# POSTECH-CVLab/InstaOrder

Measured on AMD Instinct MI355X. Metric: instance-pairs/sec (fwd+bwd), higher is better.
Workload: dtype f32; 1 GPU; InstaOrderNet_o, pair-batch 256 per GPU at 256x256x5, fp32, fwd+bwd+SGD (BASELINE.json configs[1]); inputs=resident in HBM, pairs_per_gpu=256, input_size=256, parallelism=dp1, hip_graph=True, setup_steps=0, inputs_distinct=True

## Files before the change

include/instaorder_hip.h:

```cpp
#ifndef INSTAORDER_HIP_H
#define INSTAORDER_HIP_H

#include <stddef.h>
#include <stdint.h>

#ifdef __cplusplus
extern "C" {
#endif

#define IO_OK 0
#define IO_ERR_SHAPE (-1)
#define IO_ERR_WORKSPACE (-2)
#define IO_ERR_LAUNCH (-3)
#define IO_ERR_STATE (-4)
#define IO_ERR_NODEVICE (-5)

#if !defined(__HIP__) && !defined(HIP_INCLUDE_HIP_HIP_RUNTIME_API_H)
typedef void* hipStream_t;
#endif

int io_abi_version(void);
const char* io_last_error_string(void);
int io_device_count(void);
int io_set_winograd(int on);
// ... 227 lines not shown

size_t io_bn_tile_partial_floats(int M, int C, int G);
int io_bn_bwd_coefs_dt(const void* dz, const void* y, int M, int C, int G, const float* gamma, const float* mean,
                       const float* rstd, float* dgamma, float* dbeta, float* coef, float* partial,
                       size_t partial_floats, int dtype, hipStream_t stream);
int io_bn_bwd_coefs_from_tile_partials(float* p1, float* p2, int M, int C, int G, const float* gamma, const float* mean,
                                       const float* rstd, float* dgamma, float* dbeta, float* coef, hipStream_t stream);
typedef struct io_dgrad_fused {
    const void* xb_y;
    const float* xb_coef;
    void* xb_dy_out;
    const void* add;
    const void* relu_mask;
    const void* ep_y;
    const float *ep_mean, *ep_rstd, *ep_scale, *ep_shift;
    void* ep_act_out;
    float *ep_p1, *ep_p2;
    float* wino_scratch;
    size_t wino_scratch_floats;
    const uint32_t* relu_maskbits;
} io_dgrad_fused;
int io_conv2d_dgrad_fused_dt(const void* dy, const void* wt, void* dx, int N, int H, int W, int Cin, int Cout, int R,
                             int S, int pad, int G, const io_dgrad_fused* f, int dtype, hipStream_t stream);
size_t io_conv2d_wino_scratch_floats(int Cin, int Cout);
int io_conv2d_fwd_wino(const float* x, const float* w, float* y, int N, int H, int W, int Cin, int Cout, int G,
                       const float* in_mean, const float* in_scale, const float* in_shift, const float* gamma,
                       const float* beta, float* running_mean, float* running_var, float momentum, float eps, float* mean,
                       float* rstd, float* scale, float* shift, float* workspace, size_t workspace_floats,
                       float* wino_scratch, size_t wino_floats, hipStream_t stream);
int io_conv2d_fwd_xf_dt(const void* x, const void* w, void* y, int N, int H, int W, int Cin, int Cout, int R, int S,
                        int stride, int pad, int G, const float* in_mean, const float* in_scale, const float* in_shift,
                        const float* gamma, const float* beta, float* running_mean, float* running_var, float momentum, float eps,
                        float* mean, float* rstd, float* scale, float* shift, float* workspace, size_t workspace_floats,
                        int dtype, hipStream_t stream);
int io_conv2d_fwd_resid(const float* y3, const float* identity, const float* w, float* y, float* out, int N, int H, int W,
                        int Cin, int Cout, int G, const float* in_mean, const float* in_scale, const float* in_shift,
                        const float* gamma, const float* beta, float* running_mean, float* running_var, float momentum,
                        float eps, float* mean, float* rstd, float* scale, float* shift, float* workspace,
                        size_t workspace_floats, hipStream_t stream);
int io_conv2d_fwd_resid_dt(const void* y3, const void* second, const void* w, void* y, void* out, uint32_t* out_bits, int N,
                           int H, int W, int Cin, int Cout, int G, int two, const float* ta, const float* tb, const float* tc,
                           float* tile_mean, float* tile_m2, int dtype, hipStream_t stream);
int io_set_bf16_p256_xop(int on);
int io_get_bf16_p256_xop(void);
typedef struct io_weight_desc {
    long src, dst_op, dst_t, dst_g;
// ... 176 lines not shown
```

instaorder_amd/_lib.py:

```python
import ctypes as C
import os

_HERE = os.path.dirname(os.path.abspath(__file__))
LIB_PATH = os.environ.get("IO_LIB_PATH") or os.path.join(_HERE, "libinstaorder_hip.so")
_lib = None

c_float_p = C.c_void_p


def csrc_digest():
    import glob
    import hashlib
    h = hashlib.sha256()
    files = sorted(glob.glob(os.path.join(_HERE, "csrc", "*.hip")) + glob.glob(os.path.join(_HERE, "csrc", "*.h")))
    files.append(os.path.join(os.path.dirname(_HERE), "include", "instaorder_hip.h"))
    for f in files:
        h.update(os.path.basename(f).encode())
        h.update(open(f, "rb").read())
    return h.hexdigest()[:16]


class TensorInfo(C.Structure):
    _fields_ = [("name", C.c_char * 64), ("kind", C.c_int), ("ndim", C.c_int), ("shape", C.c_long * 4),
                ("offset", C.c_long), ("numel_storage", C.c_long), ("cin_storage", C.c_int),
# ... 176 lines not shown
                                      _P, _P, _P, _P, _Z, _I, _I, _P]),
    "io_conv2d_fwd_bias_dt": (_I, [_P, _P, _P, _I, _I, _I, _I, _I, _I, _I, _I, _I, _P, _P, _I, _I, _I, _P]),
    "io_stem_packed_floats": (_Z, [_I]),
    "io_stem_wgrad_exact_workspace_bytes": (_Z, [_I, _I, _I, _I]),
    "io_stem_fwd_bnstats_exact": (_I, [_P, _P, _P, _I, _I, _I, _I, _I, _P, _P, _P, _P, _F, _F, _P, _P, _P, _P, _P, _Z, _P,
                                       _P]),
    "io_stem_wgrad_exact": (_I, [_P, _P, _P, _I, _I, _I, _I, _P, _Z, _P, _P]),
    "io_stem_wgrad_exact_bn": (_I, [_P, _P, _P, _P, _I, _I, _I, _I, _I, _P, _P, _P, _P, _P, _P, _P, _P, _P, _Z, _P, _Z, _P,
                                    _P]),
    "io_stem_wgrad_bn_bf16": (_I, [_P, _P, _P, _P, _I, _I, _I, _I, _P, _P, _P, _P, _P, _P, _P, _P, _P, _Z, _P, _Z, _P]),
    "io_stem_wgrad_bf16_workspace_bytes": (_Z, []),
    "io_debug_last_wgrad_route": (_I, []),
    "io_conv2d_fwd_resid": (_I, [_P, _P, _P, _P, _P, _I, _I, _I, _I, _I, _I, _P, _P, _P, _P, _P, _P, _P, _F, _F, _P, _P, _P,
                                 _P, _P, _Z, _P]),
    "io_smooth_loss_workspace_floats": (_Z, [_I, _I, _I]),
    "io_smooth_loss_fwd": (_I, [_P, _P, _I, _I, _I, _F, _P, _P, _P, _Z, _P]),
    "io_smooth_loss_bwd": (_I, [_P, _P, _P, _F, _I, _I, _I, _I, _P, _P]),
    "io_disp_order_workspace_floats": (_Z, [_I, _I, _I]),
    "io_disp_order_count": (_I, [_P, _P, _P, _P, _P, _P, _I, _I, _I, _I, _F, _P, _P, _Z, _P]),
    "io_bn_tile_partial_floats": (_Z, [_I, _I, _I]),
    "io_bn_bwd_coefs_dt": (_I, [_P, _P, _I, _I, _I, _P, _P, _P, _P, _P, _P, _P, _Z, _I, _P]),
    "io_bn_bwd_coefs_from_tile_partials": (_I, [_P, _P, _I, _I, _I, _P, _P, _P, _P, _P, _P, _P]),
    "io_conv2d_dgrad_fused_dt": (_I, [_P, _P, _P, _I, _I, _I, _I, _I, _I, _I, _I, _I, C.POINTER(DgradFused), _I, _P]),
    "io_conv2d_dgrad_bnbwd_dt": (_I, [_P, _P, _P, _I, _I, _I, _I, _I, _I, _I, _I, _P, _I, _P, _P, _P, _P, _P, _P, _P, _P, _P,
                                      _Z, _I, _I, _P]),
    "io_prof_launches": (_I, [_P, _I]),
    "io_weights_prepare": (_I, [_P, _I, _P, _P, _I, _P]),
    "io_weights_unpack_grads": (_I, [_P, _I, _P, _P, _P]),
    "io_maxpool_fwd_xf_dt": (_I, [_P, _I, _I, _I, _I, _P, _P, _I, _P, _P, _P, _I, _P]),
    "io_conv2d_fwd_xf_dt": (_I, [_P, _P, _P, _I, _I, _I, _I, _I, _I, _I, _I, _I, _I, _P, _P, _P, _P, _P, _P, _P, _F, _F, _P,
                                 _P, _P, _P, _P, _Z, _I, _P]),
    "io_conv2d_wino_scratch_floats": (_Z, [_I, _I]),
    "io_conv2d_fwd_wino": (_I, [_P, _P, _P, _I, _I, _I, _I, _I, _I, _P, _P, _P, _P, _P, _P, _P, _F, _F, _P, _P, _P, _P, _P, _Z,
                                _P, _Z, _P]),
    "io_maxpool_fwd_dt": (_I, [_P, _I, _I, _I, _I, _P, _P, _I, _P]),
    "io_maxpool_bwd_dt": (_I, [_P, _P, _I, _I, _I, _I, _P, _I, _P]),
    "io_avgpool_fc_fwd_dt": (_I, [_P, _I, _I, _I, _P, _P, _I, _P, _P, _I, _P, _P, _I, _P]),
    "io_avgpool_fc_bwd_dt": (_I, [_P, _P, _I, _I, _I, _P, _I, _P, _I, _P, _P, _P, _P, _P, _P, _I, _P]),
    "io_depth_errors_median_workspace_bytes": (_Z, [_I, _I, _I]),
    "io_depth_errors_median": (_I, [_P, _P, _I, _I, _I, _F, _F, _F, _P, _P, _P, _Z, _P]),
    "io_disp_sample_points": (_I, [_P, _I, _I, _I, _P, _P, _P, _P]),
    "io_mask_pack": (_I, [_P, _I, _I, _I, _I, _I, _P, _P, _P]),
    "io_mask_pair_counts": (_I, [_P, _I, _P, _I, _I, _I, _P, _P]),
    "io_instance_depth_select_workspace_bytes": (_Z, [_I, _I, _I]),
    "io_instance_depth_select": (_I, [_P, _I, _I, _P, _I, _I, _P, _P, _P, _P, _P, _Z, _P]),
    "io_prof_begin": (_I, []),
# ... 40 lines not shown
```

instaorder_amd/csrc/capi.hip:

```cpp
#include <stdarg.h>
#include <stdio.h>
#include <stdlib.h>
#include <string.h>

#include "io_common.h"

static thread_local char g_err[512] = "";

void io_set_error(const char* fmt, ...) {
    va_list ap;
    va_start(ap, fmt);
    vsnprintf(g_err, sizeof(g_err), fmt, ap);
    va_end(ap);
}

int io_check_launch(const char* what) {
    hipError_t e = hipGetLastError();
    if (e != hipSuccess) {
        io_set_error("%s: %s", what, hipGetErrorString(e));
        return IO_ERR_LAUNCH;
    }
    return IO_OK;
}

// ... 158 lines not shown
    return io_conv_wgrad_partial_bytes(g, Cin == 8);
}

extern "C" int io_conv2d_wgrad(const float* x, const float* dy, float* dw, int N, int H, int W, int Cin, int Cout,
                               int R, int S, int stride, int pad, void* ws, size_t ws_bytes, hipStream_t st) {
    IoConvGeom g = io_geom_fwd(N, H, W, Cin, Cout, R, S, stride, pad);
    return io_launch_conv_wgrad(g, x, dy, dw, (float*)ws, ws_bytes, Cin == 8, st);
}

#include <mutex>
#include <vector>
namespace {
struct ProfRec { int cls; double flops, bytes, fexec; hipEvent_t e0, e1; bool own0, closed; hipStream_t st; };
std::mutex g_prof_mu;
bool g_prof_on = false;
bool g_prof_share = true;
std::vector<ProfRec> g_prof_recs;
std::vector<hipEvent_t> g_prof_pool;
const char* kProfNames[IO_PROF_NCLASS] = {"conv_nt_kernel<128,false>", "conv_nt_kernel<64,false>",
    "conv_nt_kernel<64,true>", "conv_wgrad_kernel", "conv_wgrad_kernel<64,64,true>", "bn_stats_finalize",
    "bn_apply", "bn_bwd", "pool_head", "filter_transpose", "pack_planes", "order_loss", "sgd_momentum",
    "conv_nt_kernel<wino>", "conv_wgrad_kernel<wino>", "adam", "grad_norm", "rle_decode", "poly_fill",
    "jpeg_entropy", "jpeg_idct", "jpeg_colour", "jpeg_prog_entropy", "png_inflate", "png_unfilter", "png_pack",
    "png_par_search", "png_par_count", "png_par_store", "png_par_resolve"};
hipEvent_t prof_event() {
    if (!g_prof_pool.empty()) { hipEvent_t e = g_prof_pool.back(); g_prof_pool.pop_back(); return e; }
    hipEvent_t e;
    (void)hipEventCreate(&e);
    return e;
}
}

IoProfScope::IoProfScope(int cls, double flops, double bytes, hipStream_t stream, double flops_exec) : idx(-1), st(stream) {
    if (!g_prof_on) return;
    std::lock_guard<std::mutex> lk(g_prof_mu);
    if (!g_prof_on) return;
    ProfRec r;
    r.cls = cls; r.flops = flops; r.bytes = bytes; r.fexec = flops_exec < 0.0 ? flops : flops_exec;
    r.st = st; r.closed = false;
    if (g_prof_share && !g_prof_recs.empty() && g_prof_recs.back().closed && g_prof_recs.back().st == st) {
        r.e0 = g_prof_recs.back().e1;
        r.own0 = false;
    } else {
        r.e0 = prof_event();
        r.own0 = true;
        (void)hipEventRecord(r.e0, st);
    }
// ... 483 lines not shown
```

instaorder_amd/csrc/conv_igemm.hip:

```cpp
#include <string.h>
#include <stdlib.h>

#include "io_common.h"

namespace {

constexpr int kThreads = 256;

__device__ __forceinline__ f32x4 ld4(const float* p) { return *reinterpret_cast<const f32x4*>(p); }
template <typename T> __device__ __forceinline__ void pin(T& v) { asm volatile("" : "+v"(v)); }
__device__ __forceinline__ void st4(float* p, f32x4 v) { *reinterpret_cast<f32x4*>(p) = v; }

__device__ __forceinline__ int xcd_remap(int b, int nwg) {
    const int q = nwg >> 3, r = nwg & 7, x = b & 7, i = b >> 3;
    return (x < r ? x * (q + 1) : r * (q + 1) + (x - r) * q) + i;
}

__device__ __forceinline__ int sdiv(int n, float rd) { return (int)(((float)n + 0.5f) * rd); }
__device__ __forceinline__ int stem_kp(int wT, int cr) { return (wT * cr + 31) / 32 * 32; }
__device__ __forceinline__ int fdiv(int n, IoFastDiv f) {
    return f.shift < 0 ? n : (int)(__umulhi((unsigned)n, f.magic) >> f.shift);
}

typedef unsigned u32x4 __attribute__((ext_vector_type(4)));
// ... 2497 lines not shown

size_t io_conv_wgrad_partial_bytes(const IoConvGeom& g, int stem) {
    const int s0 = plan_wgrad(g, stem, true).splits, s1 = plan_wgrad(g, stem, false).splits;
    int splits = s0 > s1 ? s0 : s1;
    if (wgrad_wino_shape_ok(g, stem)) {
        const int sw = plan_wgrad_wino(g).splits;
        if (sw > splits) splits = sw;
    }
    size_t need = splits == 1 ? 0 : (size_t)splits * g.Co * io_filter_row(g) * sizeof(float);
    if (stem && g.cr && io_stem_rows_ok(g)) {
        const size_t rows = (size_t)io_stem_wgrad_rows_max_blocks() * g.Co * io_filter_row(g) * sizeof(float);
        if (rows > need) need = rows;
    }
    if (stem && !g.cr && g.Ci == 8 && g.Co == 64 && g.Wo == 128)
        if (io_stem_wgrad_halo_partial_bytes() > need) need = io_stem_wgrad_halo_partial_bytes();
    if (!stem && io_wgrad_halo3_shape(g) && io_wgrad_halo3_partial_bytes() > need) need = io_wgrad_halo3_partial_bytes();
    return need;
}

static std::atomic<int> g_last_wgrad_route{0};
extern "C" int io_debug_last_wgrad_route(void) { return g_last_wgrad_route.load(std::memory_order_relaxed); }
static std::atomic<int> g_last_route{0};
extern "C" int io_debug_last_nt_route(void) { return g_last_route.load(std::memory_order_relaxed); }

int io_launch_conv_nt(const IoConvGeom& g, const void* in, const void* wgt, void* out, const void* add,
                      const void* mask, int stem, hipStream_t st, float* st_mean, float* st_m2,
                      const IoBwStats* bw, int dt_in, int dt_out) {
    IoBwStats bws;
    memset(&bws, 0, sizeof(bws));
    if (bw) {
        bws = *bw;
        const long Mchk = (long)g.N * g.Ho * g.Wo;
        IO_REQUIRE(!bws.y || (g.os == 1 && g.Ho == g.outH && g.Wo == g.outW && bws.Mg > 0 && bws.Mg % 128 == 0 &&
                              Mchk % 128 == 0 && Mchk % bws.Mg == 0),
                   IO_ERR_SHAPE, "conv_nt: fused BN-backward reductions need a dense output and 128 | rows per group | M");
        IO_REQUIRE(!bws.xb_res || (bws.xb_a && !bws.y && dt_in == dt_out), IO_ERR_SHAPE,
                   "conv_nt: the residual operand form is a forward path (no BatchNorm-backward epilogue)");
        IO_REQUIRE(!bws.xb_a || (bws.xb_b && bws.xb_c && bws.xb_y && !bws.in_scale && !stem && !g.gw && g.is == 1 &&
                                 g.Hi == g.Ho && g.Wi == g.Wo &&
                                 bws.xb_Mg > 0 && bws.xb_Mg % 128 == 0 && Mchk % bws.xb_Mg == 0 && g.dhs * g.dhs == 1 &&
                                 g.dws * g.dws == 1 && g.dh0 * (g.dh0 + g.dhs * (g.Th - 1)) <= 0 &&
                                 g.dw0 * (g.dw0 + g.dws * (g.Tw - 1)) <= 0),
                   IO_ERR_SHAPE,
                   "conv_nt: the backward operand transform needs a stride-1 same-size data gradient whose taps include "
                   "the centre, and 128 | rows per group | M");
    }
// ... 417 lines not shown
```

instaorder_amd/csrc/conv_p256.hip:

```cpp
#include <stdlib.h>
#include <string.h>


#include "io_common.h"

namespace {

typedef __bf16 bf16x8 __attribute__((ext_vector_type(8)));
typedef unsigned u32x4 __attribute__((ext_vector_type(4)));
constexpr unsigned kOob = 0xFFFFFFFFu;

__device__ __forceinline__ int xcd_remap(int b, int nwg) {
    const int q = nwg >> 3, r = nwg & 7, x = b & 7, i = b >> 3;
    return (x < r ? x * (q + 1) : r * (q + 1) + (x - r) * q) + i;
}
__device__ __forceinline__ int fdiv(int n, IoFastDiv f) {
    return f.shift < 0 ? n : (int)(__umulhi((unsigned)n, f.magic) >> f.shift);
}
__device__ __forceinline__ u32x4 dma_rsrc(const void* p, size_t base, size_t total) {
    const unsigned long long a = (unsigned long long)p + base;
    const size_t rest = total > base ? total - base : 0;
    const u32x4 r = {(unsigned)a, (unsigned)(a >> 32) & 0xffffu, rest > 0xFFFFFFFFull ? 0xFFFFFFFFu : (unsigned)rest,
                     0x00020000u};
    return r;
// ... 457 lines not shown
    d.lin = g.Th * g.Tw == 1 && g.is == 1 && g.dh0 == 0 && g.dw0 == 0 && g.Hi == g.Ho && g.Wi == g.Wo;
    d.xop = bw && bw->xb_a;
    if (d.xop && (!d.lin || !env.xop || g.Ci > kXopMaxCi || !bw->xb_b || !bw->xb_c || !bw->xb_y || bw->xb_Mg <= 0 || bw->xb_Mg % 256 != 0 ||
                  M % bw->xb_Mg != 0 || add || mask || bw->maskbits || bw->bias))
        return d;
    if (st_mean && (add || mask || (bw && (bw->y || bw->bias)))) return d;
    if (bw && bw->y && (bw->Mg % 256 != 0 || bw->bias)) return d;
    if (bw && bw->y && bw->mscale && (add || mask || bw->maskbits)) return d;
    const double span = 256.0 / ((double)g.Ho * g.Wo) + 2.0;
    if (span * 2.0 * g.Hi * g.Wi * g.Ci >= 4.0e9 || 256.0 * g.Co * 2.0 >= 4.0e9) return d;
    if (g.Hi >= 32768 || g.Wi >= 32768) return d;
    d.bn = g.Co % 256 == 0 ? 256 : 128;
    d.epi = st_mean ? EPI_STATS : ((bw && bw->y) ? (bw->mscale ? EPI_BWE : EPI_BWE_READ) : EPI_PLAIN);
    d.xmode = !d.xop ? 0 : (bw->xb_res == 2 ? 3 : (bw->xb_res ? 2 : 1));
    if (d.xop && (d.epi == EPI_BWE_READ || (d.epi == EPI_BWE && d.xmode == 2))) return d;
    d.tiles = (M / 256) * (g.Co / d.bn);
    if (d.tiles >= (1L << 31) || !p256_rounds_ok(d.tiles, env)) return d;
    d.take = true;
    return d;
}

}

IoRouteEnv io_route_env_now() { return IoRouteEnv{p256_enabled(), xop_enabled(), io_device_cu_count()}; }

extern "C" int io_get_bf16_p256_xop(void) { return xop_enabled(); }
extern "C" int io_set_bf16_p256_xop(int on) {
    const int prev = xop_enabled();
    g_xop.store(on ? 1 : 0, std::memory_order_relaxed);
    return prev;
}
bool io_conv_p256_takes_xop(const IoRouteEnv& env, int N, int H, int W, int Ci, int Co, int Mg) {
    IoBwStats bw{};
    bw.xb_y = bw.xb_a = bw.xb_b = bw.xb_c = reinterpret_cast<const float*>(&bw);
    bw.xb_Mg = Mg;
    return p256_decide(io_geom_fwd(N, H, W, Ci, Co, 1, 1, 1, 0), false, false, false, &bw, env).take;
}

extern "C" int io_get_bf16_p256(void) { return p256_enabled(); }
extern "C" int io_set_bf16_p256(int on) {
    const int prev = p256_enabled();
    g_p256.store((on == 2 || on == 3) ? on : (on ? 1 : 0), std::memory_order_relaxed);
    return prev;
}
int io_bf16_persist_mode() { return p256_enabled(); }

int io_launch_conv_p256(const IoConvGeom& g, const void* in, const void* wgt, void* out, const void* add, const void* mask,
// ... 82 lines not shown
```

instaorder_amd/csrc/io_common.h:

```cpp
#pragma once
#include <hip/hip_runtime.h>
#include <stdint.h>
#include <stddef.h>

#include "../../include/instaorder_hip.h"

void io_set_error(const char* fmt, ...);
int io_check_launch(const char* what);

#define IO_REQUIRE(cond, code, ...)        \
    do {                                   \
        if (!(cond)) {                     \
            io_set_error(__VA_ARGS__);     \
            return (code);                 \
        }                                  \
    } while (0)

static inline int io_cdiv(long a, long b) { return (int)((a + b - 1) / b); }

#include <atomic>
static inline int io_device_cu_count() {
    static std::atomic<int> cache[64];
    int dev = 0;
    if (hipGetDevice(&dev) != hipSuccess || dev < 0 || dev >= 64) return 256;
// ... 93 lines not shown
    void* a_out;
    const float* bias;
    int relu;
    const float *in_mean, *in_scale, *in_shift;
    int in_Mg;
    const void* xb_y;
    const float *xb_a, *xb_b, *xb_c;
    void* xb_out;
    int xb_Mg;
    int xb_res;
    uint32_t* xb_bits;
    float* wino_u;
    const uint32_t* maskbits;
};

bool io_wino_on();

int io_launch_conv_nt(const IoConvGeom& g, const void* in, const void* wgt, void* out, const void* add,
                      const void* mask, int stem, hipStream_t st, float* st_mean = nullptr,
                      float* st_m2 = nullptr, const IoBwStats* bw = nullptr, int dt_in = IO_F32,
                      int dt_out = IO_F32);
struct IoRouteEnv {
    int p256_mode, xop, ncu;
};
IoRouteEnv io_route_env_now();
bool io_conv_p256_takes_xop(const IoRouteEnv& env, int N, int H, int W, int Ci, int Co, int Mg);
int io_launch_conv_p256(const IoConvGeom& g, const void* in, const void* wgt, void* out, const void* add, const void* mask,
                        hipStream_t st, float* st_mean, float* st_m2, const IoBwStats* bw, size_t in_bytes,
                        unsigned w_bytes, size_t out_bytes);
int io_bf16_persist_mode();
int io_launch_conv_halo3(const IoConvGeom& g, const void* in, const void* wgt, void* out, const void* add, const void* mask,
                         hipStream_t st, float* st_mean, float* st_m2, const IoBwStats* bw, size_t in_bytes,
                         unsigned w_bytes, size_t out_bytes);
int io_launch_conv_stem_halo(const IoConvGeom& g, const void* in, const void* wgt, void* out, hipStream_t st, float* st_mean,
                             float* st_m2, const IoBwStats* bw, size_t in_bytes, unsigned w_bytes, size_t out_bytes);
int io_bn_bwd_from_tiles(float* p1, float* p2, const void* dz, const void* y, int M, int C, int G,
                         const float* gamma, const float* mean, const float* rstd, float* dgamma, float* dbeta,
                         void* dy, float* coef, hipStream_t st, int dt = IO_F32);
int io_bn_bwd_coefs_from_tiles(float* p1, float* p2, int M, int C, int G, const float* gamma, const float* mean,
                               const float* rstd, float* dgamma, float* dbeta, float* coef, hipStream_t st);
int io_bn_bwd_coefs_t(const void* dz, const void* y, int M, int C, int G, const float* gamma, const float* mean,
                      const float* rstd, float* dgamma, float* dbeta, float* coef, float* partial,
                      size_t partial_floats, hipStream_t st, int dt, const float* mask_scale = nullptr,
                      const float* mask_shift = nullptr);
int io_bn_stats_finalize_t(const void* y, int M, int C, int G, const float* gamma, const float* beta,
                           float* running_mean, float* running_var, float momentum, float eps, float* mean,
// ... 39 lines not shown
    const float *y, *a, *b, *c, *mean, *scale, *shift;
    int G, tiles_per_group;
};
int io_launch_stem_wgrad_rows(const IoConvGeom& g, const float* x8, const float* dy, float* dwp, float* partial,
                              size_t partial_bytes, hipStream_t st, const IoStemXb* xb = nullptr);
size_t io_stem_wgrad_halo_partial_bytes();
bool io_stem_wgrad_halo_ok(const IoConvGeom& g, size_t partial_bytes, int G);
int io_launch_stem_wgrad_halo(const IoConvGeom& g, const void* x8, const void* dz, float* dw, float* partial, size_t partial_bytes,
                              hipStream_t st, const IoStemXb* xb);
size_t io_wgrad_halo3_partial_bytes();
bool io_wgrad_halo3_shape(const IoConvGeom& g);
int io_launch_conv_wgrad_halo3(const IoConvGeom& g, const void* x, const void* dy, float* dw, float* partial, size_t partial_bytes,
                               hipStream_t st);
int io_splitk_reduce(const float* partial, float* dst, size_t n4, int splits, hipStream_t st);
struct IoFilterTable {
    static constexpr int kMax = 64;
    int n;
    int start[kMax + 1];
    int O[kMax], T[kMax], C[kMax];
    unsigned off[kMax];
};
int io_filter_table_add(IoFilterTable& tab, long off, int O, int T, int C);
int io_filter_transpose_all(const IoFilterTable& tab, const float* params, void* wt_all, hipStream_t st, int dt);
IoConvGeom io_geom_dgrad(int N, int H, int W, int Cin, int Cout, int R, int S, int stride, int pad, int ph, int pw);
int io_run_dgrad(const void* dy, const void* wt, void* dx, const void* add, const void* mask, int N, int H,
                 int W, int Cin, int Cout, int R, int S, int stride, int pad, hipStream_t st,
                 const IoBwStats* bw = nullptr, int dt = IO_F32, int gw = 0);

enum IoProfClass {
    IO_PROF_CONV_NT128 = 0, IO_PROF_CONV_NT64, IO_PROF_CONV_STEM, IO_PROF_WGRAD, IO_PROF_WGRAD_STEM,
    IO_PROF_BN_STATS, IO_PROF_BN_APPLY, IO_PROF_BN_BWD, IO_PROF_POOL_HEAD, IO_PROF_TRANSPOSE, IO_PROF_PACK,
    IO_PROF_LOSS, IO_PROF_SGD, IO_PROF_CONV_WINO, IO_PROF_WGRAD_WINO, IO_PROF_ADAM, IO_PROF_GRAD_NORM,
    IO_PROF_RLE, IO_PROF_POLY, IO_PROF_JPEG_ENTROPY, IO_PROF_JPEG_IDCT, IO_PROF_JPEG_COLOUR, IO_PROF_JPEG_PROG_ENTROPY,
    IO_PROF_PNG_INFLATE, IO_PROF_PNG_UNFILTER, IO_PROF_PNG_PACK, IO_PROF_PNG_PAR_SEARCH, IO_PROF_PNG_PAR_COUNT,
    IO_PROF_PNG_PAR_STORE, IO_PROF_PNG_PAR_RESOLVE, IO_PROF_NCLASS
};
struct IoProfScope {
    int idx;
    hipStream_t st;
    IoProfScope(int cls, double flops, double bytes, hipStream_t stream, double flops_exec = -1.0);
    ~IoProfScope();
};
```

instaorder_amd/csrc/net.hip:

```cpp
#include <stdio.h>
#include <string.h>

#include <vector>

#include "io_common.h"

namespace {

constexpr int kMaxGroups = 8;
constexpr float kBnEps = 1e-5f, kBnMomentum = 0.1f;

struct ConvL {
    int cin, cout, k, stride, pad, cin_store;
    long w_off;
};
struct BnL {
    int C;
    long g_off, b_off, run_off;
    int index;
};
struct Block {
    ConvL c1, c2, c3, cd;
    BnL b1, b2, b3, bd;
    bool down;
// ... 153 lines not shown
            bb.bits = bits_allocated(net->dtype, Mo) ? a.take((size_t)Mo * b.planes * 4 / 8) : kNoBuf;
            H = Ho;
        }
        for (int i = 0; i < 5; ++i) p.gbuf[i] = a.take(maxact);
        p.aside = net->dtype == IO_F32 ? a.take(maxact / 2) : kNoBuf;
        size_t wg = 0, wtmax = 0;
        {
            IoConvGeom g = io_geom_fwd(N, S, S, 8, 64, 7, 7, 2, 3);
            if (net->dtype == IO_F32) g.cr = net->in_ch;
            wg = io_conv_wgrad_partial_bytes(g, 1);
        }
        H = H1;
        for (const Block& b : net->blocks) {
            const ConvL* cs[4] = {&b.c1, &b.c2, &b.c3, b.down ? &b.cd : nullptr};
            for (int j = 0; j < 4; ++j) {
                if (!cs[j]) continue;
                const ConvL& c = *cs[j];
                const int Hin = (j == 2) ? H / b.stride : H;
                IoConvGeom g = io_geom_fwd(N, Hin, Hin, c.cin, c.cout, c.k, c.k, c.stride, c.pad);
                const size_t need = io_conv_wgrad_partial_bytes(g, 0);
                if (need > wg) wg = need;
                const size_t wsz = (size_t)c.cout * c.k * c.k * c.cin * e;
                if (wsz > wtmax) wtmax = wsz;
            }
            H /= b.stride;
        }
        p.wg_partial_bytes = wg;
        p.wg_partial = a.take(wg);
        p.wt = a.take(wtmax);
        p.wt_all = a.take((size_t)net->param_floats * e);
    } else {
        const size_t r0 = a.take(maxact), r1 = a.take(maxact), r2 = a.take(maxact), r3 = a.take(maxact),
                     r4 = a.take(maxact), r5 = a.take(maxact);
        p.y0 = r3; p.a0 = r1; p.p0 = r0; p.idx0 = 0;
        size_t xin = r0, xout = r5;
        for (size_t i = 0; i < net->blocks.size(); ++i) {
            BlockBufs& bb = p.blk[i];
            bb.y1 = r3; bb.a1 = r1; bb.y2 = r3; bb.a2 = r2; bb.y3 = r3; bb.yd = r4; bb.out = xout; bb.bits = kNoBuf;
            const size_t t = xin; xin = xout; xout = t;
        }
        for (int i = 0; i < 5; ++i) p.gbuf[i] = 0;
        p.aside = kNoBuf;
        p.wg_partial = p.wt = 0;
        p.wt_all = kNoBuf;
        p.wg_partial_bytes = 0;
    }
    p.total = a.top;
    return p;
}

#ifndef IO_XB_BF16_MAXP
#define IO_XB_BF16_MAXP 64
#endif
#ifndef IO_XB_BF16_L1
#define IO_XB_BF16_L1 1
#endif
constexpr int kBwdStages = 4;
using RouteEnv = IoRouteEnv;

struct BlockRoute {
    int H, Ho, Min, Mout;
    int stage;
    bool tiles_in, tiles_out;
    bool a1_stored, a2_stored, bits_alloc;
    bool f2, f3;
    int out_route;
    bool bits_written;
    bool x3, x3p;
    bool x1d, x1s;
    bool carry;
    bool have_tiles;
};

int plan_routes(const io_net* net, int N, int S, int G, const RouteEnv& env, std::vector<BlockRoute>& out) {
    const size_t nb = net->blocks.size();
    const bool f32 = net->dtype == IO_F32;
    out.assign(nb, BlockRoute{});
    int H = S / 4, res = -1;
    for (size_t i = 0; i < nb; ++i) {
        const Block& b = net->blocks[i];
        BlockRoute& r = out[i];
        r.H = H;
        r.Ho = H / b.stride;
        r.Min = N * r.H * r.H;
        r.Mout = N * r.Ho * r.Ho;
        if (i == 0 || b.stride != 1) res += 1;
        r.stage = res;
        H = r.Ho;
        r.tiles_in = whole_tiles(r.Min, G);
        r.tiles_out = whole_tiles(r.Mout, G);
        r.a2_stored = !act_never_stored(net->dtype, r.Mout);
        r.a1_stored = r.a2_stored || b.stride != 1;
        r.bits_alloc = bits_allocated(net->dtype, r.Mout);
        r.f3 = reads_through_bn(net->dtype, r.Mout, G);
        r.f2 = r.f3 && b.stride == 1;
        IO_REQUIRE((r.f2 || r.a1_stored) && (r.f3 || r.a2_stored), IO_ERR_SHAPE,
                   "io_net_forward: G=%d does not divide this batch into whole 128-row tiles (use G in 1, 2, 4, 8)", G);
        const bool narrow = IO_XB_BF16_L1 && b.planes <= IO_XB_BF16_MAXP;
        const bool wide = !f32 && b.planes > IO_XB_BF16_MAXP && r.tiles_out;
        if (i + 1 < nb && r.tiles_out)
            r.out_route = (f32 || narrow) ? 1
                        : io_conv_p256_takes_xop(env, N, r.Ho, r.Ho, b.planes * 4, net->blocks[i + 1].planes, r.Mout / G) ? 2 : 0;
        r.bits_written = r.bits_alloc && r.out_route != 1;
        r.x3p = wide && io_conv_p256_takes_xop(env, N, r.Ho, r.Ho, b.planes * 4, b.planes, r.Mout / G);
        r.x3 = r.tiles_out && (f32 || r.x3p || narrow);
        r.x1d = b.stride == 1 && f32 && r.tiles_in && r.tiles_out;
        r.x1s = b.stride != 1 && f32 && r.tiles_in && r.a1_stored;
        r.carry = i > 0 && r.tiles_in;
        if (i > 0) out[i - 1].have_tiles = r.carry;
    }
    for (BlockRoute& r : out) r.stage = res - r.stage;
    IO_REQUIRE(res + 1 == kBwdStages, IO_ERR_STATE, "run_backward: %d resolution stages, expected %d", res + 1, kBwdStages);
    return IO_OK;
}

struct FoldDesc {
    long w_off, g_off, b_off, run_off, bias_off;
    int rows, rowlen;
};
struct FoldTable {
    int n;
    FoldDesc d[56];
};
template <typename T>
__global__ __launch_bounds__(256) void fold_bn_kernel(FoldTable t, const float* __restrict__ params,
                                                     const float* __restrict__ running, float eps,
                                                     T* __restrict__ wout, float* __restrict__ bias) {
    const FoldDesc d = t.d[blockIdx.y];
// ... 421 lines not shown
int bn_back_tiles(const Ctx& c, const BnL& b, const void* dz, const void* y, int M, void* dy) {
    Tables t = c.tables(b);
    return io_bn_bwd_from_tiles(c.buf(c.plan.tile_mean), c.buf(c.plan.tile_m2), dz, y, M, b.C, c.G,
                                c.params + b.g_off, t.mean, t.rstd, c.grads + b.g_off, c.grads + b.b_off, dy,
                                c.buf(c.plan.coef), c.st, c.dt());
}

int dgrad_then_bn(const Ctx& c, const ConvL& L, const void* dy, void* dx, int H, const BnL& b, const void* y,
                  int M, void* dyb, void* a_out = nullptr, const BnL* xb = nullptr, const void* xb_y = nullptr,
                  int xb_M = 0, void* xb_out = nullptr) {
    if (L.stride == 1 && whole_tiles(M, c.G)) {
        IoBwStats bw = bw_for(c, b, y, M, true);
        bw.a_out = a_out;
        if (xb) xb_fill(c, bw, *xb, xb_y, xb_M, xb_out);
        if (c.plan.wino_u != kNoBuf && L.k == 3 && c.dt() == IO_F32 && !xb) bw.wino_u = c.buf(c.plan.wino_u);
        IO_TRY(conv_dgrad(c, L, dy, dx, nullptr, nullptr, H, &bw));
        if (!dyb) return IO_OK;
        return bn_back_tiles(c, b, dx, y, M, dyb);
    }
    IO_REQUIRE(!xb && dyb, IO_ERR_STATE, "dgrad_then_bn: the operand transform needs the fused path");
    IO_REQUIRE(!a_out, IO_ERR_STATE, "dgrad_then_bn: no fused epilogue to rebuild the activation in");
    IO_TRY(conv_dgrad(c, L, dy, dx, nullptr, nullptr, H));
    return bn_back(c, b, dx, 1, nullptr, y, M, dyb, nullptr);
}

int stem_bn_coefs(const Ctx& c, const void* dz, IoStemXb& xb) {
    const BnL& b = c.net->bn1;
    Tables t = c.tables(b);
    IO_TRY(io_bn_bwd_coefs_t(dz, c.act(c.plan.y0), c.N * (c.S / 2) * (c.S / 2), b.C, c.G, c.params + b.g_off, t.mean, t.rstd,
                             c.grads + b.g_off, c.grads + b.b_off, c.buf(c.plan.coef), c.buf(c.plan.bn_partial),
                             c.plan.bn_partial_floats, c.st, c.dt(), t.scale, t.shift));
    const size_t gs = (size_t)c.G * b.C;
    xb = IoStemXb{};
    xb.y = (const float*)c.act(c.plan.y0);
    xb.a = c.buf(c.plan.coef);
    xb.b = c.buf(c.plan.coef) + gs;
    xb.c = c.buf(c.plan.coef) + 2 * gs;
    xb.mean = t.mean;
    xb.scale = t.scale;
    xb.shift = t.shift;
    xb.G = c.G;
    return IO_OK;
}

int run_backward(Ctx& c, const float* dlogits, const void* x8, int stage_lo = 0, int stage_hi = kBwdStages) {
    const io_net* net = c.net;
// ... 12 lines not shown
                               net->head_dims[0], w1, net->n_heads > 1 ? net->head_dims[1] : 0,
                               c.act(p.blk[nb - 1].out), dout_buf(nb - 1), c.grads + net->fcw_off[0], c.grads + net->fcb_off[0],
                               net->n_heads > 1 ? c.grads + net->fcw_off[1] : nullptr,
                               net->n_heads > 1 ? c.grads + net->fcb_off[1] : nullptr, c.st, c.dt()));
    for (size_t ii = nb; ii-- > 0;) {
        const Block& b = net->blocks[ii];
        const BlockBufs& bb = p.blk[ii];
        const BlockRoute& r = c.routes[ii];
        if (r.stage < stage_lo || r.stage >= stage_hi) continue;
        const int H = r.H, Ho = r.Ho, Min = r.Min, Mout = r.Mout;
        void *Gd = dout_buf((long)ii), *Ge = dout_buf((long)ii - 1);
        const void* xin = ii == 0 ? c.act(p.p0) : c.act(p.blk[ii - 1].out);
        const void* xmask = ii == 0 ? nullptr : xin;
        const bool x3 = r.x3, x3p = r.x3p, f3 = r.f3, f2 = r.f2, x1d = r.x1d, x1s = r.x1s;
        const bool x1 = x1d || x1s;
        if (x3)
            IO_TRY(bn_back_coefs(c, b.b3, Gd, c.act(bb.y3), Mout, r.have_tiles));
        else if (r.have_tiles)
            IO_TRY(bn_back_tiles(c, b.b3, Gd, c.act(bb.y3), Mout, Ga));
        else
            IO_TRY(bn_back(c, b.b3, Gd, 0, nullptr, c.act(bb.y3), Mout, Ga, nullptr));
        void* As = f3 ? c.act(p.aside) : nullptr;
        if (!f3 && !x3) IO_TRY(conv_wgrad(c, b.c3, c.act(bb.a2), Ga, Ho));
        IO_TRY(dgrad_then_bn(c, b.c3, x3 ? Gd : Ga, Gb, Ho, b.b2, c.act(bb.y2), Mout, Gc, f3 ? As : nullptr,
                             x3 ? &b.b3 : nullptr, c.act(bb.y3), Mout, Ga));
        if (f3 || x3) IO_TRY(conv_wgrad(c, b.c3, f3 ? As : c.act(bb.a2), Ga, Ho));
        if (!f2) IO_TRY(conv_wgrad(c, b.c2, c.act(bb.a1), Gc, H));
        if (x1s)
            IO_TRY(conv_dgrad(c, b.c2, Gc, Ga, nullptr, c.act(bb.a1), H));
        else
            IO_TRY(dgrad_then_bn(c, b.c2, Gc, Ga, H, b.b1, c.act(bb.y1), Min, x1 ? nullptr : Gb, f2 ? As : nullptr));
        if (f2) IO_TRY(conv_wgrad(c, b.c2, As, Gc, H));
        if (!x1) IO_TRY(conv_wgrad(c, b.c1, xin, Gb, H));
        const void* partial = Gd;
        if (b.down && x3 && !x3p) {
            IO_TRY(bn_back_coefs(c, b.bd, Gd, c.act(bb.yd), Mout, false));
            IoBwStats bw{};
            xb_fill(c, bw, b.bd, c.act(bb.yd), Mout, Gc);
            IO_TRY(conv_dgrad(c, b.cd, Gd, Ge, nullptr, nullptr, H, &bw));
            IO_TRY(conv_wgrad(c, b.cd, xin, Gc, H));
            partial = Ge;
        } else if (b.down) {
            IO_TRY(bn_back(c, b.bd, Gd, 0, nullptr, c.act(bb.yd), Mout, Gc, nullptr));
            IO_TRY(conv_wgrad(c, b.cd, xin, Gc, H));
            IO_TRY(conv_dgrad(c, b.cd, Gc, Ge, nullptr, nullptr, H));
            partial = Ge;
        }
        if (x1) IO_TRY(bn_back_coefs(c, b.b1, Ga, c.act(bb.y1), Min, x1d));
        {
// ... 289 lines not shown
```

Before: 1810 pairs/s.

## Fuse conv3 dgrad and wgrad into one pass for 64-plane bottleneck blocks

```diff
diff --git a/include/instaorder_hip.h b/include/instaorder_hip.h
--- a/include/instaorder_hip.h
+++ b/include/instaorder_hip.h
@@ -273,6 +273,12 @@
 } io_dgrad_fused;
 int io_conv2d_dgrad_fused_dt(const void* dy, const void* wt, void* dx, int N, int H, int W, int Cin, int Cout, int R,
                              int S, int pad, int G, const io_dgrad_fused* f, int dtype, hipStream_t stream);
+size_t io_conv2d_bwd_pair_workspace_bytes(int M, int planes);
+int io_conv2d_bwd_pair(const float* dz3, const float* y3, const float* y2, const float* wt, float* dz2, float* dw, int M,
+                       int planes, int G, const float* xb_coef, const float* mean, const float* rstd, const float* scale,
+                       const float* shift, float* p1, float* p2, float* workspace, size_t workspace_bytes, int max_blocks,
+                       hipStream_t stream);
+long io_debug_bwd_pair_launches(void);
 size_t io_conv2d_wino_scratch_floats(int Cin, int Cout);
 int io_conv2d_fwd_wino(const float* x, const float* w, float* y, int N, int H, int W, int Cin, int Cout, int G,
                        const float* in_mean, const float* in_scale, const float* in_shift, const float* gamma,
diff --git a/instaorder_amd/_lib.py b/instaorder_amd/_lib.py
--- a/instaorder_amd/_lib.py
+++ b/instaorder_amd/_lib.py
@@ -222,6 +222,9 @@
     "io_bn_bwd_coefs_dt": (_I, [_P, _P, _I, _I, _I, _P, _P, _P, _P, _P, _P, _P, _Z, _I, _P]),
     "io_bn_bwd_coefs_from_tile_partials": (_I, [_P, _P, _I, _I, _I, _P, _P, _P, _P, _P, _P, _P]),
     "io_conv2d_dgrad_fused_dt": (_I, [_P, _P, _P, _I, _I, _I, _I, _I, _I, _I, _I, _I, C.POINTER(DgradFused), _I, _P]),
+    "io_conv2d_bwd_pair_workspace_bytes": (_Z, [_I, _I]),
+    "io_conv2d_bwd_pair": (_I, [_P, _P, _P, _P, _P, _P, _I, _I, _I, _P, _P, _P, _P, _P, _P, _P, _P, _Z, _I, _P]),
+    "io_debug_bwd_pair_launches": (_L, []),
     "io_conv2d_dgrad_bnbwd_dt": (_I, [_P, _P, _P, _I, _I, _I, _I, _I, _I, _I, _I, _P, _I, _P, _P, _P, _P, _P, _P, _P, _P, _P,
                                       _Z, _I, _I, _P]),
     "io_prof_launches": (_I, [_P, _I]),
diff --git a/instaorder_amd/csrc/capi.hip b/instaorder_amd/csrc/capi.hip
--- a/instaorder_amd/csrc/capi.hip
+++ b/instaorder_amd/csrc/capi.hip
@@ -204,7 +204,7 @@
     "bn_apply", "bn_bwd", "pool_head", "filter_transpose", "pack_planes", "order_loss", "sgd_momentum",
     "conv_nt_kernel<wino>", "conv_wgrad_kernel<wino>", "adam", "grad_norm", "rle_decode", "poly_fill",
     "jpeg_entropy", "jpeg_idct", "jpeg_colour", "jpeg_prog_entropy", "png_inflate", "png_unfilter", "png_pack",
-    "png_par_search", "png_par_count", "png_par_store", "png_par_resolve"};
+    "png_par_search", "png_par_count", "png_par_store", "png_par_resolve", "conv_bwd_pair_kernel"};
 hipEvent_t prof_event() {
     if (!g_prof_pool.empty()) { hipEvent_t e = g_prof_pool.back(); g_prof_pool.pop_back(); return e; }
     hipEvent_t e;
diff --git a/instaorder_amd/csrc/conv_bwd_pair.hip b/instaorder_amd/csrc/conv_bwd_pair.hip
--- /dev/null
+++ b/instaorder_amd/csrc/conv_bwd_pair.hip
@@ -0,0 +1,268 @@
+#include <stdlib.h>
+
+#include "io_common.h"
+
+namespace {
+
+constexpr int kP = 64;
+constexpr int kK = 4 * kP;
+constexpr int kNK = kK / 32;
+constexpr int kBM = 128;
+constexpr int kLD = 36, kLY = kP + 4;
+constexpr int kMaxBlocks = 512;
+constexpr size_t kLdsBytes = (size_t)(kBM * kLD + kP * kLD + kBM * kLY + 3 * kK) * sizeof(float);
+static_assert(kBM == kIoStatTileRows, "the tile partials are per 128 rows");
+
+__device__ __forceinline__ f32x4 ld4(const float* p) { return *reinterpret_cast<const f32x4*>(p); }
+__device__ __forceinline__ void st4(float* p, f32x4 v) { *reinterpret_cast<f32x4*>(p) = v; }
+template <typename T> __device__ __forceinline__ void pin(T& v) { asm volatile("" : "+v"(v)); }
+
+struct PairArgs {
+    const float *dz3, *y3, *y2, *wt;
+    float *dz2, *partial;
+    const float *xa, *xb, *xc;
+    const float *mean, *rstd, *scale, *shift;
+    float *p1, *p2;
+    int tiles, tiles_per_group;
+};
+
+__global__ __launch_bounds__(256, 2) void conv_bwd_pair_kernel(PairArgs a) {
+    extern __shared__ __attribute__((aligned(16))) float smem[];
+    float* sD = smem;
+    float* sW = sD + kBM * kLD;
+    float* sY = sW + kP * kLD;
+    float* sC = sY + kBM * kLY;
+    const int tid = threadIdx.x, lane = tid & 63, wave = tid >> 6;
+    const int wm = wave >> 1, wn = wave & 1;
+    const int t0 = (int)((long)blockIdx.x * a.tiles / gridDim.x), t1 = (int)((long)(blockIdx.x + 1) * a.tiles / gridDim.x);
+    const int lr = tid >> 3, kq = tid & 7;
+    const int yr = tid >> 4, yc = tid & 15;
+
+    f32x4 ra[4], ry[4], rb[2];
+    auto load_k = [&](int t, int kt) {
+        const size_t base = (size_t)t * kBM * kK + (size_t)(kt * 32 + kq * 4);
+#pragma unroll
+        for (int j = 0; j < 4; ++j) {
+            ra[j] = ld4(a.dz3 + base + (size_t)(lr + 32 * j) * kK);
+            ry[j] = ld4(a.y3 + base + (size_t)(lr + 32 * j) * kK);
+        }
+#pragma unroll
+        for (int j = 0; j < 2; ++j) rb[j] = ld4(a.wt + (lr + 32 * j) * kK + kt * 32 + kq * 4);
+    };
+    auto xform = [&](int kt) {
+        const f32x4 ca = ld4(sC + kt * 32 + kq * 4), cb = ld4(sC + kK + kt * 32 + kq * 4), cc = ld4(sC + 2 * kK + kt * 32 + kq * 4);
+#pragma unroll
+        for (int j = 0; j < 4; ++j)
+#pragma unroll
+            for (int e = 0; e < 4; ++e) ra[j][e] = __builtin_fmaf(ra[j][e], ca[e], __builtin_fmaf(ry[j][e], cb[e], cc[e]));
+    };
+    auto stage_y = [&](int t) {
+        if (tid < 192) {
+            const float* tab = tid < 64 ? a.xa : (tid < 128 ? a.xb : a.xc);
+            st4(sC + tid * 4, ld4(tab + (t / a.tiles_per_group) * kK + (tid & 63) * 4));
+        }
+        f32x4 yq[8];
+#pragma unroll
+        for (int j = 0; j < 8; ++j) yq[j] = ld4(a.y2 + ((size_t)t * kBM + yr + 16 * j) * kP + yc * 4);
+#pragma unroll
+        for (int j = 0; j < 8; ++j) st4(sY + (yr + 16 * j) * kLY + yc * 4, yq[j]);
+    };
+
+    f32x4 dw[2 * kNK];
+#pragma unroll
+    for (int i = 0; i < 2 * kNK; ++i) dw[i] = f32x4{0.f, 0.f, 0.f, 0.f};
+
+    const int a_off = (wm * 64 + (lane & 31)) * kLD + (lane >> 5) * 4;
+    const int b_off = (wn * 32 + (lane & 31)) * kLD + (lane >> 5) * 4;
+    const int wcol = wave * 16 + (lane & 15);
+    const int gd_off = 4 * (lane >> 4) * kLD + (lane & 15);
+    const int gy_off = 4 * (lane >> 4) * kLY + wcol;
+    const int ecol = wn * 32 + (lane & 31);
+
+    if (t0 < t1) {
+        load_k(t0, 0);
+        stage_y(t0);
+    }
+    __syncthreads();
+    for (int t = t0; t < t1; ++t) {
+        const int gb = (t / a.tiles_per_group) * kP;
+        const float m2 = a.mean[gb + wcol], s2 = a.scale[gb + wcol], h2 = a.shift[gb + wcol];
+        f32x16 acc[2];
+#pragma unroll
+        for (int i = 0; i < 2; ++i)
+#pragma unroll
+            for (int r = 0; r < 16; ++r) acc[i][r] = 0.f;
+        xform(0);
+#pragma unroll
+        for (int kt = 0; kt < kNK; ++kt) {
+#pragma unroll
+            for (int j = 0; j < 4; ++j) st4(sD + (lr + 32 * j) * kLD + kq * 4, ra[j]);
+#pragma unroll
+            for (int j = 0; j < 2; ++j) st4(sW + (lr + 32 * j) * kLD + kq * 4, rb[j]);
+            __syncthreads();
+            if (kt + 1 < kNK) load_k(t, kt + 1);
+            else if (t + 1 < t1) load_k(t + 1, 0);
+            float qa[4], qb[4], qy[4];
+            f32x4 fa[2][2], fb[2];
+            auto wl = [&](int ks) {
+                const int p = 16 * (ks >> 2) + (ks & 3);
+                qa[ks & 3] = sD[gd_off + p * kLD];
+                qb[ks & 3] = sD[gd_off + p * kLD + 16];
+                qy[ks & 3] = sY[gy_off + p * kLY];
+            };
+            auto dl = [&](int kk) {
+#pragma unroll
+                for (int i = 0; i < 2; ++i) fa[kk & 1][i] = ld4(sD + a_off + i * 32 * kLD + kk * 8);
+                fb[kk & 1] = ld4(sW + b_off + kk * 8);
+            };
+            dl(0);
+#pragma unroll
+            for (int ks = 0; ks < 4; ++ks) wl(ks);
+            float g0 = 0.f, g1 = 0.f, gv = 0.f;
+#pragma unroll
+            for (int ks = 0; ks < 32; ++ks) {
+                g0 = qa[ks & 3];
+                g1 = qb[ks & 3];
+                gv = fmaxf(__builtin_fmaf(qy[ks & 3] - m2, s2, h2), 0.f);
+                if (ks + 4 < 32) wl(ks + 4);
+                if ((ks & 7) == 4 && ks + 4 < 32) dl((ks >> 3) + 1);
+                dw[2 * kt] = __builtin_amdgcn_mfma_f32_16x16x4f32(g0, gv, dw[2 * kt], 0, 0, 0);
+                dw[2 * kt + 1] = __builtin_amdgcn_mfma_f32_16x16x4f32(g1, gv, dw[2 * kt + 1], 0, 0, 0);
+                acc[ks & 1] = __builtin_amdgcn_mfma_f32_32x32x2f32(fa[(ks >> 3) & 1][ks & 1][(ks >> 1) & 3],
+                                                                   fb[(ks >> 3) & 1][(ks >> 1) & 3], acc[ks & 1], 0, 0, 0);
+                __builtin_amdgcn_sched_barrier(0);
+            }
+            if (kt + 1 < kNK) xform(kt + 1);
+            pin(fa[1][0]); pin(fa[1][1]); pin(fb[1]); pin(g0); pin(g1); pin(gv);
+            __syncthreads();
+        }
+
+        {
+            const float mu = a.mean[gb + ecol], rs = a.rstd[gb + ecol], sc = a.scale[gb + ecol], sh = a.shift[gb + ecol];
+            float s1 = 0.f, sx = 0.f;
+            float* const orow = a.dz2 + (size_t)t * kBM * kP + ecol;
+#pragma unroll
+            for (int i = 0; i < 2; ++i) {
+                float yv[16];
+#pragma unroll
+                for (int r = 0; r < 16; ++r)
+                    yv[r] = sY[(wm * 64 + i * 32 + (r & 3) + 8 * (r >> 2) + 4 * (lane >> 5)) * kLY + ecol];
+#pragma unroll
+                for (int r = 0; r < 16; ++r) {
+                    const int row = wm * 64 + i * 32 + (r & 3) + 8 * (r >> 2) + 4 * (lane >> 5);
+                    float v = acc[i][r] + 0.f;
+                    const float tn = __builtin_fmaf(yv[r] - mu, sc, sh);
+                    v = tn > 0.f ? v : 0.f;
+                    s1 += v;
+                    sx += v * ((yv[r] - mu) * rs);
+                    __builtin_nontemporal_store(v, orow + (size_t)row * kP);
+                }
+            }
+            float* red = sD;
+            const float ua = s1 + __shfl_xor(s1, 32, 64);
+            const float ub = sx + __shfl_xor(sx, 32, 64);
+            if (lane < 32) {
+                red[wm * kP + ecol] = ua;
+                red[2 * kP + wm * kP + ecol] = ub;
+            }
+            __syncthreads();
+            if (t + 1 < t1) stage_y(t + 1);
+            if (wm == 0 && lane < 32) {
+                const size_t o = (size_t)t * kP + ecol;
+                a.p1[o] = red[ecol] + red[kP + ecol];
+                a.p2[o] = red[2 * kP + ecol] + red[3 * kP + ecol];
+            }
+            __syncthreads();
+        }
+    }
+
+    float* const slab = a.partial + (size_t)blockIdx.x * kK * kP;
+#pragma unroll
+    for (int i = 0; i < 2 * kNK; ++i)
+#pragma unroll
+        for (int r = 0; r < 4; ++r) slab[(i * 16 + 4 * (lane >> 4) + r) * kP + wcol] = dw[i][r];
+}
+
+std::atomic<int> g_pair_on{-1};
+std::atomic<long> g_pair_launches{0};
+
+}
+
+int io_bwd_pair_enabled() {
+    int on = g_pair_on.load(std::memory_order_relaxed);
+    if (on < 0) {
+        const char* e = getenv("IO_BWD_PAIR");
+        on = (e && e[0] == '0') ? 0 : 1;
+        g_pair_on.store(on, std::memory_order_relaxed);
+    }
+    return on;
+}
+
+int io_conv_bwd_pair_grid(long M, int ncu, int max_blocks) {
+    long grid = M / kBM;
+    if (grid > 2L * ncu) grid = 2L * ncu;
+    if (grid > kMaxBlocks) grid = kMaxBlocks;
+    if (max_blocks > 0 && grid > max_blocks) grid = max_blocks;
+    return (int)grid;
+}
+size_t io_conv_bwd_pair_partial_bytes(long M, int planes) {
+    if (planes != kP || M < kBM) return 0;
+    const long tiles = M / kBM;
+    return (size_t)(tiles < kMaxBlocks ? tiles : kMaxBlocks) * kK * kP * sizeof(float);
+}
+bool io_conv_bwd_pair_takes(long M, int planes, int G) {
+    return planes == kP && G >= 1 && M > 0 && M % G == 0 && (M / G) % kBM == 0 && M / kBM < (1L << 24);
+}
+
+bool io_conv_bwd_pair_pays(long M, int ncu) { return ncu >= 1 && M / kBM >= 4L * ncu; }
+
+extern "C" long io_debug_bwd_pair_launches(void) { return g_pair_launches.load(std::memory_order_relaxed); }
+
+int io_launch_conv_bwd_pair(const float* dz3, const float* y3, const float* y2, const float* wt, float* dz2, float* dw,
+                            long M, int planes, int G, const float* xb_coef, const float* mean, const float* rstd,
+                            const float* scale, const float* shift, float* p1, float* p2, float* partial,
+                            size_t partial_bytes, int max_blocks, hipStream_t st) {
+    IO_REQUIRE(planes == kP, IO_ERR_SHAPE, "conv_bwd_pair: planes=%d (this kernel holds the filter gradient of %d planes)",
+               planes, kP);
+    IO_REQUIRE(io_conv_bwd_pair_takes(M, planes, G), IO_ERR_SHAPE,
+               "conv_bwd_pair: M=%ld rows in G=%d groups must be whole %d-row tiles per group", M, G, kBM);
+    IO_REQUIRE(dz3 && y3 && y2 && wt && dz2 && dw && xb_coef && mean && rstd && scale && shift && p1 && p2 && partial,
+               IO_ERR_SHAPE, "conv_bwd_pair: null argument");
+    IO_REQUIRE(max_blocks >= 0, IO_ERR_SHAPE, "conv_bwd_pair: max_blocks=%d", max_blocks);
+    const int grid = io_conv_bwd_pair_grid(M, io_device_cu_count(), max_blocks);
+    const size_t slab = (size_t)kK * kP * sizeof(float);
+    IO_REQUIRE(partial_bytes >= (size_t)grid * slab, IO_ERR_WORKSPACE, "conv_bwd_pair: partial buffer %zu < %zu bytes",
+               partial_bytes, (size_t)grid * slab);
+    static std::atomic<unsigned long long> attr_done{0};
+    if (io_first_on_device(attr_done))
+        (void)hipFuncSetAttribute((const void*)conv_bwd_pair_kernel, hipFuncAttributeMaxDynamicSharedMemorySize,
+                                  (int)kLdsBytes);
+    PairArgs a;
+    a.dz3 = dz3; a.y3 = y3; a.y2 = y2; a.wt = wt;
+    a.dz2 = dz2; a.partial = partial;
+    const size_t gs = (size_t)G * kK;
+    a.xa = xb_coef; a.xb = xb_coef + gs; a.xc = xb_coef + 2 * gs;
+    a.mean = mean; a.rstd = rstd; a.scale = scale; a.shift = shift;
+    a.p1 = p1; a.p2 = p2;
+    a.tiles = (int)(M / kBM);
+    a.tiles_per_group = (int)(M / G / kBM);
+    {
+        IoProfScope prof(IO_PROF_BWD_PAIR, 2.0 * 2.0 * (double)M * kK * kP,
+                         4.0 * ((double)M * (2.0 * kK + 2.0 * kP) + (double)kK * kP * (1.0 + grid)), st);
+        hipLaunchKernelGGL(conv_bwd_pair_kernel, dim3(grid), dim3(256), kLdsBytes, st, a);
+    }
+    g_pair_launches.fetch_add(1, std::memory_order_relaxed);
+    io_debug_set_nt_route(4);
+    int rc = io_check_launch("conv_bwd_pair");
+    if (rc) return rc;
+    return io_splitk_reduce(partial, dw, (size_t)kK * kP / 4, grid, st);
+}
+
+extern "C" int io_conv2d_bwd_pair(const float* dz3, const float* y3, const float* y2, const float* wt, float* dz2, float* dw,
+                                  int M, int planes, int G, const float* xb_coef, const float* mean, const float* rstd,
+                                  const float* scale, const float* shift, float* p1, float* p2, float* workspace,
+                                  size_t workspace_bytes, int max_blocks, hipStream_t st) {
+    return io_launch_conv_bwd_pair(dz3, y3, y2, wt, dz2, dw, M, planes, G, xb_coef, mean, rstd, scale, shift, p1, p2,
+                                   workspace, workspace_bytes, max_blocks, st);
+}
+extern "C" size_t io_conv2d_bwd_pair_workspace_bytes(int M, int planes) { return io_conv_bwd_pair_partial_bytes(M, planes); }
diff --git a/instaorder_amd/csrc/conv_igemm.hip b/instaorder_amd/csrc/conv_igemm.hip
--- a/instaorder_amd/csrc/conv_igemm.hip
+++ b/instaorder_amd/csrc/conv_igemm.hip
@@ -2543,6 +2543,7 @@
 extern "C" int io_debug_last_wgrad_route(void) { return g_last_wgrad_route.load(std::memory_order_relaxed); }
 static std::atomic<int> g_last_route{0};
 extern "C" int io_debug_last_nt_route(void) { return g_last_route.load(std::memory_order_relaxed); }
+void io_debug_set_nt_route(int route) { g_last_route.store(route, std::memory_order_relaxed); }
 
 int io_launch_conv_nt(const IoConvGeom& g, const void* in, const void* wgt, void* out, const void* add,
                       const void* mask, int stem, hipStream_t st, float* st_mean, float* st_m2,
diff --git a/instaorder_amd/csrc/conv_p256.hip b/instaorder_amd/csrc/conv_p256.hip
--- a/instaorder_amd/csrc/conv_p256.hip
+++ b/instaorder_amd/csrc/conv_p256.hip
@@ -503,7 +503,7 @@
 
 }
 
-IoRouteEnv io_route_env_now() { return IoRouteEnv{p256_enabled(), xop_enabled(), io_device_cu_count()}; }
+IoRouteEnv io_route_env_now() { return IoRouteEnv{p256_enabled(), xop_enabled(), io_device_cu_count(), io_bwd_pair_enabled()}; }
 
 extern "C" int io_get_bf16_p256_xop(void) { return xop_enabled(); }
 extern "C" int io_set_bf16_p256_xop(int on) {
diff --git a/instaorder_amd/csrc/io_common.h b/instaorder_amd/csrc/io_common.h
--- a/instaorder_amd/csrc/io_common.h
+++ b/instaorder_amd/csrc/io_common.h
@@ -139,6 +139,7 @@
                       int dt_out = IO_F32);
 struct IoRouteEnv {
     int p256_mode, xop, ncu;
+    int pair;
 };
 IoRouteEnv io_route_env_now();
 bool io_conv_p256_takes_xop(const IoRouteEnv& env, int N, int H, int W, int Ci, int Co, int Mg);
@@ -224,6 +225,15 @@
 };
 int io_filter_table_add(IoFilterTable& tab, long off, int O, int T, int C);
 int io_filter_transpose_all(const IoFilterTable& tab, const float* params, void* wt_all, hipStream_t st, int dt);
+bool io_conv_bwd_pair_takes(long M, int planes, int G);
+bool io_conv_bwd_pair_pays(long M, int ncu);
+size_t io_conv_bwd_pair_partial_bytes(long M, int planes);
+int io_bwd_pair_enabled();
+int io_launch_conv_bwd_pair(const float* dz3, const float* y3, const float* y2, const float* wt, float* dz2, float* dw,
+                            long M, int planes, int G, const float* xb_coef, const float* mean, const float* rstd,
+                            const float* scale, const float* shift, float* p1, float* p2, float* partial,
+                            size_t partial_bytes, int max_blocks, hipStream_t st);
+void io_debug_set_nt_route(int route);
 IoConvGeom io_geom_dgrad(int N, int H, int W, int Cin, int Cout, int R, int S, int stride, int pad, int ph, int pw);
 int io_run_dgrad(const void* dy, const void* wt, void* dx, const void* add, const void* mask, int N, int H,
                  int W, int Cin, int Cout, int R, int S, int stride, int pad, hipStream_t st,
@@ -235,7 +245,7 @@
     IO_PROF_LOSS, IO_PROF_SGD, IO_PROF_CONV_WINO, IO_PROF_WGRAD_WINO, IO_PROF_ADAM, IO_PROF_GRAD_NORM,
     IO_PROF_RLE, IO_PROF_POLY, IO_PROF_JPEG_ENTROPY, IO_PROF_JPEG_IDCT, IO_PROF_JPEG_COLOUR, IO_PROF_JPEG_PROG_ENTROPY,
     IO_PROF_PNG_INFLATE, IO_PROF_PNG_UNFILTER, IO_PROF_PNG_PACK, IO_PROF_PNG_PAR_SEARCH, IO_PROF_PNG_PAR_COUNT,
-    IO_PROF_PNG_PAR_STORE, IO_PROF_PNG_PAR_RESOLVE, IO_PROF_NCLASS
+    IO_PROF_PNG_PAR_STORE, IO_PROF_PNG_PAR_RESOLVE, IO_PROF_BWD_PAIR, IO_PROF_NCLASS
 };
 struct IoProfScope {
     int idx;
diff --git a/instaorder_amd/csrc/net.hip b/instaorder_amd/csrc/net.hip
--- a/instaorder_amd/csrc/net.hip
+++ b/instaorder_amd/csrc/net.hip
@@ -199,6 +199,10 @@
                 if (need > wg) wg = need;
                 const size_t wsz = (size_t)c.cout * c.k * c.k * c.cin * e;
                 if (wsz > wtmax) wtmax = wsz;
+                if (j == 2 && net->dtype == IO_F32) {
+                    const size_t pair = io_conv_bwd_pair_partial_bytes((long)N * Hin * Hin, b.planes);
+                    if (pair > wg) wg = pair;
+                }
             }
             H /= b.stride;
         }
@@ -244,6 +248,7 @@
     int out_route;
     bool bits_written;
     bool x3, x3p;
+    bool pair3;
     bool x1d, x1s;
     bool carry;
     bool have_tiles;
@@ -281,6 +286,8 @@
         r.bits_written = r.bits_alloc && r.out_route != 1;
         r.x3p = wide && io_conv_p256_takes_xop(env, N, r.Ho, r.Ho, b.planes * 4, b.planes, r.Mout / G);
         r.x3 = r.tiles_out && (f32 || r.x3p || narrow);
+        r.pair3 = env.pair && f32 && r.x3 && r.f3 && r.tiles_out && b.planes <= 128 &&
+                  io_conv_bwd_pair_takes(r.Mout, b.planes, G) && io_conv_bwd_pair_pays(r.Mout, env.ncu);
         r.x1d = b.stride == 1 && f32 && r.tiles_in && r.tiles_out;
         r.x1s = b.stride != 1 && f32 && r.tiles_in && r.a1_stored;
         r.carry = i > 0 && r.tiles_in;
@@ -748,6 +755,16 @@
     IO_REQUIRE(!a_out, IO_ERR_STATE, "dgrad_then_bn: no fused epilogue to rebuild the activation in");
     IO_TRY(conv_dgrad(c, L, dy, dx, nullptr, nullptr, H));
     return bn_back(c, b, dx, 1, nullptr, y, M, dyb, nullptr);
+}
+
+int conv3_bwd_pair(const Ctx& c, const Block& b, const void* dz3, const void* y3, const void* y2, void* dz2, int M) {
+    IO_REQUIRE(c.dt() == IO_F32 && c.plan.wt_all != kNoBuf, IO_ERR_STATE, "conv3_bwd_pair: an fp32 training plan is required");
+    Tables t = c.tables(b.b2);
+    const float* wt = reinterpret_cast<const float*>(c.act(c.plan.wt_all)) + b.c3.w_off;
+    return io_launch_conv_bwd_pair((const float*)dz3, (const float*)y3, (const float*)y2, wt, (float*)dz2,
+                                   c.grads + b.c3.w_off, M, b.planes, c.G, c.buf(c.plan.coef), t.mean, t.rstd, t.scale,
+                                   t.shift, c.buf(c.plan.tile_mean), c.buf(c.plan.tile_m2), c.buf(c.plan.wg_partial),
+                                   c.plan.wg_partial_bytes, 0, c.st);
 }
 
 int stem_bn_coefs(const Ctx& c, const void* dz, IoStemXb& xb) {
@@ -806,9 +823,14 @@
             IO_TRY(bn_back(c, b.b3, Gd, 0, nullptr, c.act(bb.y3), Mout, Ga, nullptr));
         void* As = f3 ? c.act(p.aside) : nullptr;
         if (!f3 && !x3) IO_TRY(conv_wgrad(c, b.c3, c.act(bb.a2), Ga, Ho));
-        IO_TRY(dgrad_then_bn(c, b.c3, x3 ? Gd : Ga, Gb, Ho, b.b2, c.act(bb.y2), Mout, Gc, f3 ? As : nullptr,
-                             x3 ? &b.b3 : nullptr, c.act(bb.y3), Mout, Ga));
-        if (f3 || x3) IO_TRY(conv_wgrad(c, b.c3, f3 ? As : c.act(bb.a2), Ga, Ho));
+        if (r.pair3) {
+            IO_TRY(conv3_bwd_pair(c, b, Gd, c.act(bb.y3), c.act(bb.y2), Gb, Mout));
+            IO_TRY(bn_back_tiles(c, b.b2, Gb, c.act(bb.y2), Mout, Gc));
+        } else {
+            IO_TRY(dgrad_then_bn(c, b.c3, x3 ? Gd : Ga, Gb, Ho, b.b2, c.act(bb.y2), Mout, Gc, f3 ? As : nullptr,
+                                 x3 ? &b.b3 : nullptr, c.act(bb.y3), Mout, Ga));
+            if (f3 || x3) IO_TRY(conv_wgrad(c, b.c3, f3 ? As : c.act(bb.a2), Ga, Ho));
+        }
         if (!f2) IO_TRY(conv_wgrad(c, b.c2, c.act(bb.a1), Gc, H));
         if (x1s)
             IO_TRY(conv_dgrad(c, b.c2, Gc, Ga, nullptr, c.act(bb.a1), H));
```

Result: no change. 1832 pairs/s (median of 4 runs) (+1.2%).
